# LanceZPF/loongx

Hardware: AMD Instinct MI355X
Metric: edited images/s @512x512, 28-step Flux denoise (higher is better)
Workload: dtype bf16

## Files before the change

loongx_amd/csrc/gemm4.h:

```cpp
#pragma once
#include "gemm_common.h"

namespace {

constexpr int G4_STAGE = 256 * BK * 2 + BN * BK * 2;
constexpr int G4_LDS = 2 * G4_STAGE;
constexpr int G4_PLD = 132;
static_assert(G4_LDS <= 160 * 1024 && 4 * 2 * 16 * G4_PLD * 4 <= G4_LDS, "LDS budget / epilogue patches");

#ifdef LX_G4_PROBE
__device__ unsigned long long lx_g4_probe_buf[8192 * 8];
#define G4_STAMP(k) if (threadIdx.x == 0 && blockIdx.x < 8192) { asm volatile("s_waitcnt lgkmcnt(0)" ::: "memory"); lx_g4_probe_buf[blockIdx.x * 8 + (k)] = __builtin_amdgcn_s_memtime(); }
#else
#define G4_STAMP(k)
#endif


template <bool SPLIT, bool F16 = false, int NP = 2>
__global__ __launch_bounds__(G4_THREADS) void lx_gemm4_kernel(const GemmArgs args, const int sk_full, const int sk_parts, float* __restrict__ sk_slots,
                                                              int* __restrict__ sk_flags, int* __restrict__ sk_err) {
#if defined(__HIP_DEVICE_COMPILE__)
  __shared__ __attribute__((aligned(1024))) char smem[G4_LDS];
  constexpr int BM = 256, A_BYTES = BM * BK * 2;
  const int pid = blockIdx.x;
  G4_STAMP(0)
  const int total = args.tile_start[MAX_SUB];
  int lid, part = 0;
  if (pid < sk_full) {
    const int q = sk_full >> 3, r = sk_full & 7;
    const int xcd = pid & 7, inx = pid >> 3;
    lid = (xcd < r ? xcd * (q + 1) : r * (q + 1) + (xcd - r) * q) + inx;
  } else {
    const int r = pid - sk_full;
    lid = sk_full + r / NP;
    part = r % NP;
  }
  (void)total;
  const bool split_tile = pid >= sk_full && sk_parts >= 2;
  const int g = tile_group(args, lid);
  lx_gemm_desc P = args.p[g];
  int tm, tn;
  tile_coords<BM>(P, lid - args.tile_start[g], tm, tn);
  const int tid = threadIdx.x, lane = tid & 63;
  const int wave = __builtin_amdgcn_readfirstlane(tid >> 6);
  const int wm = wave >> 1, wn = wave & 1, l15 = lane & 15, lq = lane >> 4;
  int m0 = tm * BM, n0 = tn * BN;
  int M = P.M, N = P.N;
  const int K = P.K;
  const bool w_tiled = (P.epilogue & LX_W_TILED) != 0;
  const int nk1 = K / BK;
  const int nkt = SPLIT ? nk1 * max(P.k_segs, 1) : nk1;
  const int kt_begin = !split_tile ? 0 : NP == 2 ? (part ? nkt >> 1 : 0) : (part * nkt) / NP;
  const int kt_end = !split_tile ? nkt : NP == 2 ? (part ? nkt : nkt >> 1) : ((part + 1) * nkt) / NP;

  uint32_t aoff[8], woff[8];
  {
    const int rsub = lane >> 3, pslot = lane & 7;
#pragma unroll
    for (int j = 0; j < 8; ++j) {
      const int row = (j * 4 + wave) * 8 + rsub;
      const int lslot = pslot ^ ((row >> 1) & 7);
      aoff[j] = (uint32_t)((min(m0 + row, M - 1) - m0) * P.lda + lslot * 8) * 2u;
      woff[j] = w_tiled ? (uint32_t)((j * 4 + wave) * 512 + lane * 8) * 2u : (uint32_t)((min(n0 + row, N - 1) - n0) * P.ldw + lslot * 8) * 2u;
    }
  }
  const __bf16* a_org = (const __bf16*)P.A + (size_t)m0 * P.lda;
  const int kw_tiles = SPLIT && P.k_segs == 3 ? 2 * nk1 : nk1;
  const __bf16* w_org = w_tiled ? (const __bf16*)P.W + ((size_t)tn * kw_tiles) * (BN * BK) : (const __bf16*)P.W + (size_t)n0 * P.ldw;
  const lx_rsrc_t rs_a = lx_make_rsrc(a_org), rs_w = lx_make_rsrc(w_org);
  const int w_kstride_b = (w_tiled ? BN * BK : BK) * 2;
  const int a_lo_b = SPLIT ? P.a_lo_off * 2 : 0;
  auto a_soff = [&](int t) -> int {
    if constexpr (!SPLIT) return t * (BK * 2);
    else {
      const int seg = t >= 2 * nk1 ? 2 : (t >= nk1 ? 1 : 0);
      return (t - seg * nk1) * (BK * 2) + (seg == 1 ? a_lo_b : 0);
    }
  };
  auto w_soff = [&](int t) -> int {
    if constexpr (!SPLIT) return t * w_kstride_b;
    else {
      const int seg = t >= 2 * nk1 ? 2 : (t >= nk1 ? 1 : 0);
      return (t - seg * nk1 + (seg == 2 ? nk1 : 0)) * w_kstride_b;
    }
  };
  auto piece = [&](int p_, int a_so, int w_so, int stage) {
    if (p_ < 8) lx_buf_to_lds(rs_a, (lptr_t)(smem + stage * G4_STAGE + (p_ * 4 + wave) * 1024), aoff[p_], a_so);
    else lx_buf_to_lds(rs_w, (lptr_t)(smem + stage * G4_STAGE + A_BYTES + ((p_ - 8) * 4 + wave) * 1024), woff[p_ - 8], w_so);
  };
  int a_ad[2], w_ad[2];
  {
    const int ar = wm * 128 + l15, wr = wn * 128 + l15;
#pragma unroll
    for (int ks = 0; ks < 2; ++ks) {
      a_ad[ks] = ar * 128 + (((ks * 4 + lq) ^ ((ar >> 1) & 7)) * 16);
      w_ad[ks] = A_BYTES + wr * 128 + (((ks * 4 + lq) ^ ((wr >> 1) & 7)) * 16);
    }
  }
  f32x4 acc[8][8];
#pragma unroll
  for (int i = 0; i < 8; ++i)
#pragma unroll
    for (int j = 0; j < 8; ++j) acc[i][j] = f32x4{0.f, 0.f, 0.f, 0.f};
  bf16x8 af[2][8], wf[2][8];
  auto rd = [&](int stage, int ks, int idx) {
    const char* base = smem + stage * G4_STAGE;
    if (idx < 8) wf[ks][idx] = *(const bf16x8*)(base + w_ad[ks] + idx * 2048);
    else af[ks][idx - 8] = *(const bf16x8*)(base + a_ad[ks] + (idx - 8) * 2048);
  };
  auto mm = [&](int ks, int n_) {
    const int j = n_ >> 3, i = n_ & 7;
    if constexpr (F16) asm volatile("v_mfma_f32_16x16x32_f16 %0, %1, %2, %0" : "+a"(acc[i][j]) : "v"(wf[ks][j]), "v"(af[ks][i]));
    else asm volatile("v_mfma_f32_16x16x32_bf16 %0, %1, %2, %0" : "+a"(acc[i][j]) : "v"(wf[ks][j]), "v"(af[ks][i]));
  };
#define G4_SB() __builtin_amdgcn_sched_barrier(0)
  const bool has_lora = P.lora_t != nullptr && kt_begin == 0;
  u32x2 lu[8], lt[8][4];
  if (has_lora) {
    const int R = P.lora_r, nsplit = P.lora_nsplit;
    const int toff = R * min(n0 / max(P.lora_mod_cols, 1), P.lora_toff_max);
    const int rk = min(2 * lq, R - 2);
#pragma unroll
    for (int j = 0; j < 8; ++j) lu[j] = *(const u32x2*)(P.lora_up + (size_t)min(n0 + wn * 128 + j * 16 + l15, N - 1) * R + rk);
#pragma unroll
    for (int i = 0; i < 8; ++i) {
      const float* tp = P.lora_t + (size_t)min(m0 + wm * 128 + i * 16 + l15, M - 1) * P.lora_ldt + toff + rk;
#pragma unroll
      for (int q = 0; q < 4; ++q) lt[i][q] = *(const u32x2*)(tp + (size_t)min(q, nsplit - 1) * P.lora_split_stride);
    }
  }
  {
    const int t1 = min(kt_begin + 1, kt_end - 1);
    const int a0 = a_soff(kt_begin), w0 = w_soff(kt_begin), a1 = a_soff(t1), w1 = w_soff(t1);
#pragma unroll
    for (int p_ = 0; p_ < 16; ++p_) piece(p_, a0, w0, 0);
#pragma unroll
    for (int p_ = 0; p_ < 16; ++p_) piece(p_, a1, w1, 1);
  }
  asm volatile("s_waitcnt vmcnt(16)" ::: "memory");
  __builtin_amdgcn_s_barrier();
  G4_SB();
  G4_STAMP(1)
#pragma unroll
  for (int x = 0; x < 16; ++x) rd(0, 0, x);
  if (has_lora) {
    const int R = P.lora_r, nsplit = P.lora_nsplit;
    const bool live = 2 * lq < R;
    auto frag_u = [&](u32x2 v) {
      const float a = live ? __uint_as_float(v[0]) : 0.f, b = live ? __uint_as_float(v[1]) : 0.f;
      const uint16_t ah = f32_to_bf16(a), bh = f32_to_bf16(b);
      const uint16_t al = f32_to_bf16(a - bf16_to_f32(ah)), bl = f32_to_bf16(b - bf16_to_f32(bh));
      const u32x4 w = {(uint32_t)ah * 0x10001u, (uint32_t)al * 0x10001u, (uint32_t)bh * 0x10001u, (uint32_t)bl * 0x10001u};
      return __builtin_bit_cast(bf16x8, w);
    };
    auto frag_t = [&](float a, float b) {
      a = live ? a : 0.f; b = live ? b : 0.f;
      const uint16_t ah = f32_to_bf16(a), bh = f32_to_bf16(b);
      const uint32_t pa = (uint32_t)ah | ((uint32_t)f32_to_bf16(a - bf16_to_f32(ah)) << 16);
      const uint32_t pb = (uint32_t)bh | ((uint32_t)f32_to_bf16(b - bf16_to_f32(bh)) << 16);
      const u32x4 w = {pa, pa, pb, pb};
      return __builtin_bit_cast(bf16x8, w);
    };
    bf16x8 uf[8], tf[8];
#pragma unroll
    for (int j = 0; j < 8; ++j) uf[j] = frag_u(lu[j]);
#pragma unroll
    for (int i = 0; i < 8; ++i) {
      float a = __uint_as_float(lt[i][0][0]), b = __uint_as_float(lt[i][0][1]);
#pragma unroll
      for (int q = 1; q < 4; ++q)
        if (q < nsplit) { a += __uint_as_float(lt[i][q][0]); b += __uint_as_float(lt[i][q][1]); }
      tf[i] = frag_t(a, b);
    }
#pragma unroll
    for (int j = 0; j < 8; ++j)
#pragma unroll
      for (int i = 0; i < 8; ++i) acc[i][j] = __builtin_amdgcn_mfma_f32_16x16x32_bf16(uf[j], tf[i], acc[i][j], 0, 0, 0);
    asm volatile("s_nop 15\n s_nop 7" ::: "memory");
  }
  asm volatile("s_waitcnt lgkmcnt(0)" ::: "memory");
  G4_STAMP(2)
  int c = 0;
  for (int kt = kt_begin; kt < kt_end; ++kt) {
    const int n = c ^ 1;
    const int kt2 = min(kt + 2, kt_end - 1);
    const int a_so2 = a_soff(kt2), w_so2 = w_soff(kt2);
#pragma unroll
    for (int m = 0; m < 64; ++m) {
      if (m == 16) {
        G4_SB();
        asm volatile("s_waitcnt lgkmcnt(0)" ::: "memory");
        __builtin_amdgcn_s_barrier();
        G4_SB();
      }
      mm(0, m); G4_SB();
      if (m < 16) { rd(c, 1, m); G4_SB(); }
      if (m >= 16 && (m - 16) % 6 == 0) { piece((m - 16) / 6, a_so2, w_so2, c); G4_SB(); }
    }
#pragma unroll
    for (int m = 0; m < 64; ++m) {
      if (m == 43) {
        G4_SB();
        asm volatile("s_waitcnt vmcnt(16)" ::: "memory");
        __builtin_amdgcn_s_barrier();
        G4_SB();
      }
      mm(1, m); G4_SB();
      if (m < 40 && m % 5 == 0) { piece(8 + m / 5, a_so2, w_so2, c); G4_SB(); }
      if (m >= 43 && m < 59) { rd(n, 0, m - 43); G4_SB(); }
    }
    asm volatile("s_waitcnt lgkmcnt(0)" ::: "memory");
    c = n;
  }
#undef G4_SB
  G4_STAMP(3)
  asm volatile("s_nop 15\n s_nop 7\n s_waitcnt vmcnt(0)" ::: "memory");
  __syncthreads();
  G4_STAMP(4)

  const float* partner = nullptr;
  const float* partner2 = nullptr;
  float* my_slot = nullptr;
  if (split_tile) {
    my_slot = sk_slots + (size_t)(pid - sk_full) * SK_SLOT_FLOATS;
    if constexpr (NP == 2) {
      partner = sk_slots + (size_t)((pid - sk_full) ^ 1) * SK_SLOT_FLOATS;
    } else {
      const int gb = (pid - sk_full) - part;
      partner = sk_slots + (size_t)(gb + (part + 1) % NP) * SK_SLOT_FLOATS;
      partner2 = sk_slots + (size_t)(gb + (part + 2) % NP) * SK_SLOT_FLOATS;
    }
  }
  auto pld4 = [&](size_t off_floats, const float* from) {
    const u32x4 v = __builtin_amdgcn_raw_buffer_load_b128(lx_make_rsrc(from), (int)(off_floats * 4), 0, PAIR_AUX_SC1);
    return f32x4{__uint_as_float(v[0]), __uint_as_float(v[1]), __uint_as_float(v[2]), __uint_as_float(v[3])};
  };
  const int lm0 = wm * 128, ln0 = wn * 128;
  auto exchange = [&]() {
    asm volatile("s_waitcnt vmcnt(0)" ::: "memory");
    __syncthreads();
    __builtin_amdgcn_fence(__ATOMIC_RELEASE, "workgroup");
    if (tid == 0) {
      const int me = pid - sk_full, other = NP == 2 ? (me ^ 1) : (me - part + (part + 1) % NP), other2 = me - part + (part + 2) % NP;
      bool ok = __hip_atomic_load(sk_err, __ATOMIC_RELAXED, __HIP_MEMORY_SCOPE_AGENT) == 0;
      if (ok) {
        if (!(sk_parts == 3 && part == 1))
          __hip_atomic_store(sk_flags + me, NP - 1, __ATOMIC_RELAXED, __HIP_MEMORY_SCOPE_AGENT);
        int spins = 0;
        while (__hip_atomic_load(sk_flags + other, __ATOMIC_RELAXED, __HIP_MEMORY_SCOPE_AGENT) == 0) {
          __builtin_amdgcn_s_sleep(1);
          if (++spins > (1 << 20)) { ok = false; break; }
        }
        if constexpr (NP == 3) {
          while (ok && __hip_atomic_load(sk_flags + other2, __ATOMIC_RELAXED, __HIP_MEMORY_SCOPE_AGENT) == 0) {
            __builtin_amdgcn_s_sleep(1);
            if (++spins > (1 << 20)) { ok = false; break; }
          }
        }
        if (ok) {
          if constexpr (NP == 2) __hip_atomic_store(sk_flags + other, 0, __ATOMIC_RELAXED, __HIP_MEMORY_SCOPE_AGENT);
          else {
            __hip_atomic_fetch_add(sk_flags + other, -1, __ATOMIC_RELAXED, __HIP_MEMORY_SCOPE_AGENT);
            __hip_atomic_fetch_add(sk_flags + other2, -1, __ATOMIC_RELAXED, __HIP_MEMORY_SCOPE_AGENT);
          }
        } else __hip_atomic_store(sk_err, 1, __ATOMIC_RELAXED, __HIP_MEMORY_SCOPE_AGENT);
      }
    }
    __syncthreads();
    G4_STAMP(6)
    __builtin_amdgcn_fence(__ATOMIC_ACQUIRE, "workgroup");
  };

  const int epi = P.epilogue & 0xff;
  const bool do_gelu = (P.epilogue & LX_EPI_GELU) != 0;
  const int mw0 = m0 + wm * 128, nw0 = n0 + wn * 128;
  float* patch = (float*)smem + wave * (2 * 16 * G4_PLD);
  const bool bf16_out = epi == LX_EPI_STORE_BF16;
  const int c8 = (lane & 15) * 8, c4 = (lane & 31) * 4;
  const int ncol = nw0 + (bf16_out ? c8 : c4);
  const bool col_ok = ncol < N;
  f32x4 bias0 = {0.f, 0.f, 0.f, 0.f}, bias1 = {0.f, 0.f, 0.f, 0.f};
  if (P.bias && col_ok) {
    bias0 = *(const f32x4*)(P.bias + ncol);
    if (bf16_out) bias1 = *(const f32x4*)(P.bias + ncol + 4);
  }
  asm volatile("s_waitcnt vmcnt(0)" : "+v"(bias0), "+v"(bias1)::"memory");
  const bool gelu0 = do_gelu && ncol >= P.gelu_col_start;
  const int m_base = args.m_base[g];
  static_assert(!(F16 && SPLIT), "fp16 operands exclude the split-bf16 mode");
  float f16_mx = 0.f;
  const bool qkv_tile = (P.epilogue & LX_EPI_QKV) != 0 && n0 < 3 * P.qkv_d;
  const int qkind = qkv_tile ? n0 / P.qkv_d : -1;
  f32x4 nw0v = {1.f, 1.f, 1.f, 1.f}, nw1v = {1.f, 1.f, 1.f, 1.f};
  if (qkv_tile && qkind != 1) {
    const float* nwp = (qkind == 2 ? P.qkv_norm_q : P.qkv_norm_k) + c8;
    nw0v = *(const f32x4*)nwp; nw1v = *(const f32x4*)(nwp + 4);
    asm volatile("s_waitcnt vmcnt(0)" : "+v"(nw0v), "+v"(nw1v)::"memory");
  }
  auto put = [&](auto ic_) {
    constexpr int i = decltype(ic_)::value;
    float* pt = patch + (i & 1) * (16 * G4_PLD);
    asm volatile("" : "+a"(acc[i][0]), "+a"(acc[i][1]), "+a"(acc[i][2]), "+a"(acc[i][3]), "+a"(acc[i][4]), "+a"(acc[i][5]), "+a"(acc[i][6]), "+a"(acc[i][7]));
#pragma unroll
    for (int j = 0; j < 8; ++j) *(f32x4*)(pt + l15 * G4_PLD + j * 16 + 4 * lq) = acc[i][j];
  };
  auto park = [&](auto ic_, auto nx_) {
    constexpr int i = decltype(ic_)::value, nx = decltype(nx_)::value;
    const float* pt = patch + (i & 1) * (16 * G4_PLD);
    __builtin_amdgcn_wave_barrier();
    if constexpr (nx >= 0) { if (mw0 + nx * 16 < M) put(std::integral_constant<int, nx>{}); }
    __builtin_amdgcn_sched_barrier(0);
    if (mw0 + i * 16 >= M) return;
    const lx_rsrc_t rs_slot = lx_make_rsrc(my_slot);
#pragma unroll
    for (int t = 0; t < 8; ++t) {
      const int row = t * 2 + (lane >> 5);
      const f32x4 v = *(const f32x4*)(pt + row * G4_PLD + c4);
      __builtin_amdgcn_raw_buffer_store_b128(u32x4{__float_as_uint(v[0]), __float_as_uint(v[1]), __float_as_uint(v[2]), __float_as_uint(v[3])}, rs_slot,
                                             (int)(((size_t)(wm * 128 + i * 16 + row) * 256 + wn * 128 + c4) * 4), 0, PAIR_AUX_SC1);
    }
  };
  auto block = [&](auto ic_, auto nx_) {
    constexpr int i = decltype(ic_)::value, nx = decltype(nx_)::value;
    const int mb = mw0 + i * 16;
    if (mb >= M) return;
    const float* pt = patch + (i & 1) * (16 * G4_PLD);
    f32x4 res[8], gat[8];
    if (epi == LX_EPI_RESID_F32 && !qkv_tile) {
      const int rpb = P.rows_per_batch;
#pragma unroll
      for (int t = 0; t < 8; ++t) {
        const int m = mb + t * 2 + (lane >> 5);
        if (m < M && col_ok) {
          res[t] = *(const f32x4*)((const float*)P.C + (size_t)m * P.ldc + ncol);
          if (P.gate) gat[t] = *(const f32x4*)(P.gate + (size_t)((m_base + m) / rpb) * P.gate_ld + ncol);
        }
      }
    }
    __builtin_amdgcn_wave_barrier();
    if constexpr (nx >= 0) { if (mw0 + nx * 16 < M) put(std::integral_constant<int, nx>{}); }
    __builtin_amdgcn_sched_barrier(0);
    if (partner) {
      f32x4 pa[4][2], pb[4][2];
#pragma unroll
      for (int t = 0; t < 4; ++t) {
        const size_t po = (size_t)(lm0 + i * 16 + t * 4 + (lane >> 4)) * 256 + ln0 + c8;
        pa[t][0] = pld4(po, partner); pa[t][1] = pld4(po + 4, partner);
        if constexpr (NP == 3) { pb[t][0] = pld4(po, partner2); pb[t][1] = pld4(po + 4, partner2); }
      }
      float* pw = patch + (i & 1) * (16 * G4_PLD);
#pragma unroll
      for (int t = 0; t < 4; ++t) {
        float* q_ = pw + (t * 4 + (lane >> 4)) * G4_PLD + c8;
        f32x4 v0 = *(const f32x4*)q_, v1 = *(const f32x4*)(q_ + 4);
#pragma unroll
        for (int c_ = 0; c_ < 4; ++c_) { v0[c_] += pa[t][0][c_]; v1[c_] += pa[t][1][c_]; }
        if constexpr (NP == 3) {
#pragma unroll
          for (int c_ = 0; c_ < 4; ++c_) { v0[c_] += pb[t][0][c_]; v1[c_] += pb[t][1][c_]; }
        }
        *(f32x4*)q_ = v0; *(f32x4*)(q_ + 4) = v1;
      }
      __builtin_amdgcn_wave_barrier();
    }
    if (qkv_tile) {
      const int D = P.qkv_d, L = P.rows_per_batch, H = D >> 7;
      const int gm = m_base + mb, b = gm / L, p0 = gm - b * L;
      const int h = (nw0 - qkind * D) >> 7;
      if (qkind == 1) {
        const int gk = lane & 1;
        float e[4][8];
#pragma unroll
        for (int t = 0; t < 4; ++t)
#pragma unroll
          for (int k = 0; k < 8; ++k) {
            const int rk = qkv_vt_interleave(gk * 8 + k), dk = t * 32 + (lane >> 1);
            e[t][k] = pt[rk * G4_PLD + dk];
          }
#pragma unroll
        for (int t = 0; t < 4; ++t) {
          const int d = t * 32 + (lane >> 1);
          const float bd = P.bias ? P.bias[nw0 + d] : 0.f;
          u32x4 o = {pack_bf16x2(e[t][0] + bd, e[t][1] + bd), pack_bf16x2(e[t][2] + bd, e[t][3] + bd), pack_bf16x2(e[t][4] + bd, e[t][5] + bd),
                     pack_bf16x2(e[t][6] + bd, e[t][7] + bd)};
          *(u32x4*)((uint16_t*)P.qkv_vt + ((size_t)(b * H + h) * 128 + d) * P.qkv_vt_ld + P.qkv_vt_pos0 + p0 + gk * 8) = o;
        }
      } else {
        uint16_t* const out = (qkind == 0 && P.qkv_k) ? (uint16_t*)P.qkv_k : (uint16_t*)P.C;
        const int out_ld = (qkind == 0 && P.qkv_k) ? P.qkv_k_ld : P.ldc;
        f32x4 cs[4][2], pv[4][2];
#pragma unroll
        for (int t = 0; t < 4; ++t) {
          const float* rp = P.qkv_rope + (size_t)(p0 + t * 4 + (lane >> 4)) * 128 + c8;
          cs[t][0] = *(const f32x4*)rp; cs[t][1] = *(const f32x4*)(rp + 4);
        }
#pragma unroll
        for (int t = 0; t < 4; ++t) {
          const int row = t * 4 + (lane >> 4);
          pv[t][0] = *(const f32x4*)(pt + row * G4_PLD + c8); pv[t][1] = *(const f32x4*)(pt + row * G4_PLD + c8 + 4);
        }
        float yy[4][8];
#pragma unroll
        for (int t = 0; t < 4; ++t) {
          f32x4 v0 = pv[t][0], v1 = pv[t][1];
          float ss = 0.f;
#pragma unroll
          for (int c_ = 0; c_ < 4; ++c_) { v0[c_] += bias0[c_]; v1[c_] += bias1[c_]; ss = __builtin_fmaf(v0[c_], v0[c_], ss); ss = __builtin_fmaf(v1[c_], v1[c_], ss); }
#ifdef LX_G4_ROW16_SHFL
          ss += __shfl_xor(ss, 1, 64); ss += __shfl_xor(ss, 2, 64); ss += __shfl_xor(ss, 4, 64); ss += __shfl_xor(ss, 8, 64);
#else
          ss = row16_sum(ss);
#endif
          const float r = rsqrtf(ss * (1.0f / 128.0f) + 1e-6f);
          float x[8];
          float (&y)[8] = yy[t];
#pragma unroll
          for (int c_ = 0; c_ < 4; ++c_) { x[c_] = v0[c_] * r * nw0v[c_]; x[4 + c_] = v1[c_] * r * nw1v[c_]; }
#pragma unroll
          for (int q = 0; q < 4; ++q) {
            const float co = q < 2 ? cs[t][0][2 * q] : cs[t][1][2 * q - 4], si = q < 2 ? cs[t][0][2 * q + 1] : cs[t][1][2 * q - 3];
            y[2 * q] = x[2 * q] * co - x[2 * q + 1] * si;
            y[2 * q + 1] = x[2 * q + 1] * co + x[2 * q] * si;
          }
        }
#pragma unroll
        for (int t = 0; t < 4; ++t) {
          const int m = mb + t * 4 + (lane >> 4);
          const float (&y)[8] = yy[t];
          u32x4 o = {pack_bf16x2(y[0], y[1]), pack_bf16x2(y[2], y[3]), pack_bf16x2(y[4], y[5]), pack_bf16x2(y[6], y[7])};
          if (m < M) *(u32x4*)(out + (size_t)m * out_ld + ncol) = o;
        }
      }
      return;
    }
    if (bf16_out) {
      f32x4 pv[4][2];
#pragma unroll
      for (int t = 0; t < 4; ++t) {
        const int row = t * 4 + (lane >> 4);
        pv[t][0] = *(const f32x4*)(pt + row * G4_PLD + c8); pv[t][1] = *(const f32x4*)(pt + row * G4_PLD + c8 + 4);
      }
#pragma unroll
      for (int t = 0; t < 4; ++t) {
        const int row = t * 4 + (lane >> 4), m = mb + row;
        f32x4 v0 = pv[t][0], v1 = pv[t][1];
        if (m < M && col_ok) {
#pragma unroll
          for (int c_ = 0; c_ < 4; ++c_) { v0[c_] += bias0[c_]; v1[c_] += bias1[c_]; }
          if (gelu0) { v0 = gelu_tanh4(v0); v1 = gelu_tanh4(v1); }
          u32x4 o = {pack_op16x2<F16>(v0[0], v0[1], f16_mx), pack_op16x2<F16>(v0[2], v0[3], f16_mx), pack_op16x2<F16>(v1[0], v1[1], f16_mx),
                     pack_op16x2<F16>(v1[2], v1[3], f16_mx)};
          *(u32x4*)((uint16_t*)P.C + (size_t)m * P.ldc + ncol) = o;
          if constexpr (SPLIT) {
            if (P.epilogue & LX_EPI_SPLIT_BF16) {
              float r[8];
#pragma unroll
              for (int c_ = 0; c_ < 4; ++c_) {
                r[c_] = v0[c_] - bf16_to_f32(f32_to_bf16(v0[c_]));
                r[4 + c_] = v1[c_] - bf16_to_f32(f32_to_bf16(v1[c_]));
              }
              u32x4 ol = {pack_bf16x2(r[0], r[1]), pack_bf16x2(r[2], r[3]), pack_bf16x2(r[4], r[5]), pack_bf16x2(r[6], r[7])};
              *(u32x4*)((uint16_t*)P.C + (size_t)m * P.ldc + ncol + P.c_lo_off) = ol;
            }
          }
        }
      }
    } else {
      f32x4 pv[8];
#pragma unroll
      for (int t = 0; t < 8; ++t) pv[t] = *(const f32x4*)(pt + (t * 2 + (lane >> 5)) * G4_PLD + c4);
      if (epi == LX_EPI_RESID_F32) {
        asm volatile("s_waitcnt vmcnt(0)" ::: "memory");
#pragma unroll
        for (int t = 0; t < 8; ++t) asm volatile("" : "+v"(res[t]), "+v"(gat[t]));
      }
#pragma unroll
      for (int t = 0; t < 8; ++t) {
        const int row = t * 2 + (lane >> 5), m = mb + row;
        f32x4 v = pv[t];
        if (m < M && col_ok) {
#pragma unroll
          for (int c_ = 0; c_ < 4; ++c_) v[c_] += bias0[c_];
          if (gelu0) v = gelu_tanh4(v);
          if (epi == LX_EPI_RESID_F32) {
            f32x4 o = res[t];
            if (P.gate) {
#pragma unroll
              for (int c_ = 0; c_ < 4; ++c_) o[c_] = __builtin_fmaf(gat[t][c_], v[c_], o[c_]);
            } else {
#pragma unroll
              for (int c_ = 0; c_ < 4; ++c_) o[c_] += v[c_];
            }
            v = o;
          }
          *(f32x4*)((float*)P.C + (size_t)m * P.ldc + ncol) = v;
        }
      }
    }
  };
#define G4_B(I, NX) block(std::integral_constant<int, I>{}, std::integral_constant<int, NX>{})
#define G4_K(I, NX) park(std::integral_constant<int, I>{}, std::integral_constant<int, NX>{})
  if (!split_tile) {
    if (mw0 < M) put(std::integral_constant<int, 0>{});
    G4_B(0, 1); G4_B(1, 2); G4_B(2, 3); G4_B(3, 4); G4_B(4, 5); G4_B(5, 6); G4_B(6, 7); G4_B(7, -1);
  } else if constexpr (NP == 2) {
    if (part == 0) {
      if (mw0 + 64 < M) put(std::integral_constant<int, 4>{});
      G4_K(4, 5); G4_K(5, 6); G4_K(6, 7); G4_K(7, 0);
      exchange();
      G4_B(0, 1); G4_B(1, 2); G4_B(2, 3); G4_B(3, -1);
    } else {
      if (mw0 < M) put(std::integral_constant<int, 0>{});
      G4_K(0, 1); G4_K(1, 2); G4_K(2, 3); G4_K(3, 4);
      exchange();
      G4_B(4, 5); G4_B(5, 6); G4_B(6, 7); G4_B(7, -1);
    }
  } else {
    if (part == 0) {
      if (mw0 + 48 < M) put(std::integral_constant<int, 3>{});
      G4_K(3, 4); G4_K(4, 5); G4_K(5, 6); G4_K(6, 7); G4_K(7, 0);
      exchange();
      G4_B(0, 1); G4_B(1, 2); G4_B(2, -1);
    } else if (part == 1) {
      if (mw0 < M) put(std::integral_constant<int, 0>{});
      G4_K(0, 1); G4_K(1, 2); G4_K(2, 7); G4_K(7, 6); G4_K(6, 3);
      exchange();
      G4_B(3, 4); G4_B(4, 5); G4_B(5, -1);
    } else {
      if (mw0 < M) put(std::integral_constant<int, 0>{});
      G4_K(0, 1); G4_K(1, 2); G4_K(2, 3); G4_K(3, 4); G4_K(4, 5); G4_K(5, 6);
      exchange();
      G4_B(6, 7); G4_B(7, -1);
    }
  }
#undef G4_B
#undef G4_K
  if constexpr (F16) { if (bf16_out && !qkv_tile) report_f16_overflow(f16_mx, P.f16_ovf); }
  asm volatile("s_waitcnt vmcnt(0)" ::: "memory");
  G4_STAMP(5)
#endif
}


}
```

Before: 1.066.

## Prefetch epilogue operands before main loop and preload first block's residual/rope

Moves the bias, qk-norm weight, V-transpose bias and per-batch gate loads ahead of the K loop so their latency hides behind the MFMA work. It also issues the first epilogue block's residual or rope loads before the post-loop barrier. Per-row gate loads are replaced with at most two hoisted gate vectors plus a fallback for tiles spanning more batches. This costs extra live VGPRs across the main loop, which could raise register pressure or spill.

Result: no change. 1.071 (median of 6 runs) (+0.5%).

```diff
diff --git a/loongx_amd/csrc/gemm4.h b/loongx_amd/csrc/gemm4.h
--- a/loongx_amd/csrc/gemm4.h
+++ b/loongx_amd/csrc/gemm4.h
@@ -127,6 +127,43 @@
       const float* tp = P.lora_t + (size_t)min(m0 + wm * 128 + i * 16 + l15, M - 1) * P.lora_ldt + toff + rk;
 #pragma unroll
       for (int q = 0; q < 4; ++q) lt[i][q] = *(const u32x2*)(tp + (size_t)min(q, nsplit - 1) * P.lora_split_stride);
+    }
+  }
+  const int epi = P.epilogue & 0xff;
+  const int mw0 = m0 + wm * 128, nw0 = n0 + wn * 128;
+  const bool bf16_out = epi == LX_EPI_STORE_BF16;
+  const int c8 = (lane & 15) * 8, c4 = (lane & 31) * 4;
+  const int ncol = nw0 + (bf16_out ? c8 : c4);
+  const bool col_ok = ncol < N;
+  const int m_base = args.m_base[g];
+  const bool qkv_tile = (P.epilogue & LX_EPI_QKV) != 0 && n0 < 3 * P.qkv_d;
+  const int qkind = qkv_tile ? n0 / P.qkv_d : -1;
+  f32x4 bias0 = {0.f, 0.f, 0.f, 0.f}, bias1 = {0.f, 0.f, 0.f, 0.f};
+  if (P.bias && col_ok) {
+    bias0 = *(const f32x4*)(P.bias + ncol);
+    if (bf16_out) bias1 = *(const f32x4*)(P.bias + ncol + 4);
+  }
+  f32x4 nw0v = {1.f, 1.f, 1.f, 1.f}, nw1v = {1.f, 1.f, 1.f, 1.f};
+  if (qkv_tile && qkind != 1) {
+    const float* nwp = (qkind == 2 ? P.qkv_norm_q : P.qkv_norm_k) + c8;
+    nw0v = *(const f32x4*)nwp; nw1v = *(const f32x4*)(nwp + 4);
+  }
+  f32x4 vtb = {0.f, 0.f, 0.f, 0.f};
+  if (qkv_tile && qkind == 1 && P.bias) {
+#pragma unroll
+    for (int t = 0; t < 4; ++t) vtb[t] = P.bias[nw0 + t * 32 + (lane >> 1)];
+  }
+  f32x4 gate0 = {0.f, 0.f, 0.f, 0.f}, gate1 = {0.f, 0.f, 0.f, 0.f};
+  int gate_edge = 0, gate_edge2 = 0;
+  bool gate_far = false;
+  if (epi == LX_EPI_RESID_F32 && !qkv_tile && P.gate && mw0 < M) {
+    const int rpb = P.rows_per_batch, b0 = (m_base + mw0) / rpb, mlast = min(mw0 + 127, M - 1);
+    gate_edge = mw0 + min(rpb - (m_base + mw0 - b0 * rpb), 256);
+    gate_edge2 = gate_edge + min(rpb, 256);
+    gate_far = mlast >= gate_edge2;
+    if (col_ok) {
+      gate0 = *(const f32x4*)(P.gate + (size_t)b0 * P.gate_ld + ncol);
+      if (mlast >= gate_edge) gate1 = *(const f32x4*)(P.gate + (size_t)(b0 + 1) * P.gate_ld + ncol);
     }
   }
   {
@@ -214,8 +251,26 @@
   }
 #undef G4_SB
   G4_STAMP(3)
-  asm volatile("s_nop 15\n s_nop 7\n s_waitcnt vmcnt(0)" ::: "memory");
-  __syncthreads();
+  asm volatile("s_waitcnt vmcnt(0)" : "+v"(bias0), "+v"(bias1), "+v"(nw0v), "+v"(nw1v), "+v"(vtb), "+v"(gate0), "+v"(gate1)::"memory");
+  const int blk_first = !split_tile ? 0 : NP == 2 ? part * 4 : part * 3;
+  const int mb_first = mw0 + blk_first * 16;
+  f32x4 pre[8];
+  if (mb_first < M) {
+    if (epi == LX_EPI_RESID_F32 && !qkv_tile) {
+#pragma unroll
+      for (int t = 0; t < 8; ++t) pre[t] = *(const f32x4*)((const float*)P.C + (size_t)min(mb_first + t * 2 + (lane >> 5), M - 1) * P.ldc + (col_ok ? ncol : n0));
+    } else if (qkv_tile && qkind != 1) {
+      const int gm = m_base + mb_first, p0 = gm - (gm / P.rows_per_batch) * P.rows_per_batch;
+#pragma unroll
+      for (int t = 0; t < 4; ++t) {
+        const float* rp = P.qkv_rope + (size_t)(p0 + t * 4 + (lane >> 4)) * 128 + c8;
+        pre[2 * t] = *(const f32x4*)rp; pre[2 * t + 1] = *(const f32x4*)(rp + 4);
+      }
+    }
+  }
+  asm volatile("s_nop 15\n s_nop 7" ::: "memory");
+  __builtin_amdgcn_s_barrier();
+  asm volatile("" ::: "memory");
   G4_STAMP(4)
 
   const float* partner = nullptr;
@@ -271,32 +326,11 @@
     __builtin_amdgcn_fence(__ATOMIC_ACQUIRE, "workgroup");
   };
 
-  const int epi = P.epilogue & 0xff;
   const bool do_gelu = (P.epilogue & LX_EPI_GELU) != 0;
-  const int mw0 = m0 + wm * 128, nw0 = n0 + wn * 128;
   float* patch = (float*)smem + wave * (2 * 16 * G4_PLD);
-  const bool bf16_out = epi == LX_EPI_STORE_BF16;
-  const int c8 = (lane & 15) * 8, c4 = (lane & 31) * 4;
-  const int ncol = nw0 + (bf16_out ? c8 : c4);
-  const bool col_ok = ncol < N;
-  f32x4 bias0 = {0.f, 0.f, 0.f, 0.f}, bias1 = {0.f, 0.f, 0.f, 0.f};
-  if (P.bias && col_ok) {
-    bias0 = *(const f32x4*)(P.bias + ncol);
-    if (bf16_out) bias1 = *(const f32x4*)(P.bias + ncol + 4);
-  }
-  asm volatile("s_waitcnt vmcnt(0)" : "+v"(bias0), "+v"(bias1)::"memory");
   const bool gelu0 = do_gelu && ncol >= P.gelu_col_start;
-  const int m_base = args.m_base[g];
   static_assert(!(F16 && SPLIT), "fp16 operands exclude the split-bf16 mode");
   float f16_mx = 0.f;
-  const bool qkv_tile = (P.epilogue & LX_EPI_QKV) != 0 && n0 < 3 * P.qkv_d;
-  const int qkind = qkv_tile ? n0 / P.qkv_d : -1;
-  f32x4 nw0v = {1.f, 1.f, 1.f, 1.f}, nw1v = {1.f, 1.f, 1.f, 1.f};
-  if (qkv_tile && qkind != 1) {
-    const float* nwp = (qkind == 2 ? P.qkv_norm_q : P.qkv_norm_k) + c8;
-    nw0v = *(const f32x4*)nwp; nw1v = *(const f32x4*)(nwp + 4);
-    asm volatile("s_waitcnt vmcnt(0)" : "+v"(nw0v), "+v"(nw1v)::"memory");
-  }
   auto put = [&](auto ic_) {
     constexpr int i = decltype(ic_)::value;
     float* pt = patch + (i & 1) * (16 * G4_PLD);
@@ -320,20 +354,20 @@
                                              (int)(((size_t)(wm * 128 + i * 16 + row) * 256 + wn * 128 + c4) * 4), 0, PAIR_AUX_SC1);
     }
   };
-  auto block = [&](auto ic_, auto nx_) {
+  auto block = [&](auto ic_, auto nx_, auto first_) {
     constexpr int i = decltype(ic_)::value, nx = decltype(nx_)::value;
+    constexpr bool first = decltype(first_)::value;
     const int mb = mw0 + i * 16;
     if (mb >= M) return;
     const float* pt = patch + (i & 1) * (16 * G4_PLD);
-    f32x4 res[8], gat[8];
+    f32x4 res[8];
     if (epi == LX_EPI_RESID_F32 && !qkv_tile) {
-      const int rpb = P.rows_per_batch;
 #pragma unroll
       for (int t = 0; t < 8; ++t) {
         const int m = mb + t * 2 + (lane >> 5);
         if (m < M && col_ok) {
-          res[t] = *(const f32x4*)((const float*)P.C + (size_t)m * P.ldc + ncol);
-          if (P.gate) gat[t] = *(const f32x4*)(P.gate + (size_t)((m_base + m) / rpb) * P.gate_ld + ncol);
+          if constexpr (first) res[t] = pre[t];
+          else res[t] = *(const f32x4*)((const float*)P.C + (size_t)m * P.ldc + ncol);
         }
       }
     }
@@ -380,7 +414,7 @@
 #pragma unroll
         for (int t = 0; t < 4; ++t) {
           const int d = t * 32 + (lane >> 1);
-          const float bd = P.bias ? P.bias[nw0 + d] : 0.f;
+          const float bd = vtb[t];
           u32x4 o = {pack_bf16x2(e[t][0] + bd, e[t][1] + bd), pack_bf16x2(e[t][2] + bd, e[t][3] + bd), pack_bf16x2(e[t][4] + bd, e[t][5] + bd),
                      pack_bf16x2(e[t][6] + bd, e[t][7] + bd)};
           *(u32x4*)((uint16_t*)P.qkv_vt + ((size_t)(b * H + h) * 128 + d) * P.qkv_vt_ld + P.qkv_vt_pos0 + p0 + gk * 8) = o;
@@ -391,8 +425,11 @@
         f32x4 cs[4][2], pv[4][2];
 #pragma unroll
         for (int t = 0; t < 4; ++t) {
-          const float* rp = P.qkv_rope + (size_t)(p0 + t * 4 + (lane >> 4)) * 128 + c8;
-          cs[t][0] = *(const f32x4*)rp; cs[t][1] = *(const f32x4*)(rp + 4);
+          if constexpr (first) { cs[t][0] = pre[2 * t]; cs[t][1] = pre[2 * t + 1]; }
+          else {
+            const float* rp = P.qkv_rope + (size_t)(p0 + t * 4 + (lane >> 4)) * 128 + c8;
+            cs[t][0] = *(const f32x4*)rp; cs[t][1] = *(const f32x4*)(rp + 4);
+          }
         }
 #pragma unroll
         for (int t = 0; t < 4; ++t) {
@@ -472,7 +509,7 @@
       if (epi == LX_EPI_RESID_F32) {
         asm volatile("s_waitcnt vmcnt(0)" ::: "memory");
 #pragma unroll
-        for (int t = 0; t < 8; ++t) asm volatile("" : "+v"(res[t]), "+v"(gat[t]));
+        for (int t = 0; t < 8; ++t) asm volatile("" : "+v"(res[t]));
       }
 #pragma unroll
       for (int t = 0; t < 8; ++t) {
@@ -485,8 +522,10 @@
           if (epi == LX_EPI_RESID_F32) {
             f32x4 o = res[t];
             if (P.gate) {
-#pragma unroll
-              for (int c_ = 0; c_ < 4; ++c_) o[c_] = __builtin_fmaf(gat[t][c_], v[c_], o[c_]);
+              f32x4 gt = m < gate_edge ? gate0 : gate1;
+              if (gate_far && m >= gate_edge2) gt = *(const f32x4*)(P.gate + (size_t)((m_base + m) / P.rows_per_batch) * P.gate_ld + ncol);
+#pragma unroll
+              for (int c_ = 0; c_ < 4; ++c_) o[c_] = __builtin_fmaf(gt[c_], v[c_], o[c_]);
             } else {
 #pragma unroll
               for (int c_ = 0; c_ < 4; ++c_) o[c_] += v[c_];
@@ -498,42 +537,44 @@
       }
     }
   };
-#define G4_B(I, NX) block(std::integral_constant<int, I>{}, std::integral_constant<int, NX>{})
+#define G4_B(I, NX) block(std::integral_constant<int, I>{}, std::integral_constant<int, NX>{}, std::false_type{})
+#define G4_F(I, NX) block(std::integral_constant<int, I>{}, std::integral_constant<int, NX>{}, std::true_type{})
 #define G4_K(I, NX) park(std::integral_constant<int, I>{}, std::integral_constant<int, NX>{})
   if (!split_tile) {
     if (mw0 < M) put(std::integral_constant<int, 0>{});
-    G4_B(0, 1); G4_B(1, 2); G4_B(2, 3); G4_B(3, 4); G4_B(4, 5); G4_B(5, 6); G4_B(6, 7); G4_B(7, -1);
+    G4_F(0, 1); G4_B(1, 2); G4_B(2, 3); G4_B(3, 4); G4_B(4, 5); G4_B(5, 6); G4_B(6, 7); G4_B(7, -1);
   } else if constexpr (NP == 2) {
     if (part == 0) {
       if (mw0 + 64 < M) put(std::integral_constant<int, 4>{});
       G4_K(4, 5); G4_K(5, 6); G4_K(6, 7); G4_K(7, 0);
       exchange();
-      G4_B(0, 1); G4_B(1, 2); G4_B(2, 3); G4_B(3, -1);
+      G4_F(0, 1); G4_B(1, 2); G4_B(2, 3); G4_B(3, -1);
     } else {
       if (mw0 < M) put(std::integral_constant<int, 0>{});
       G4_K(0, 1); G4_K(1, 2); G4_K(2, 3); G4_K(3, 4);
       exchange();
-      G4_B(4, 5); G4_B(5, 6); G4_B(6, 7); G4_B(7, -1);
+      G4_F(4, 5); G4_B(5, 6); G4_B(6, 7); G4_B(7, -1);
     }
   } else {
     if (part == 0) {
       if (mw0 + 48 < M) put(std::integral_constant<int, 3>{});
       G4_K(3, 4); G4_K(4, 5); G4_K(5, 6); G4_K(6, 7); G4_K(7, 0);
       exchange();
-      G4_B(0, 1); G4_B(1, 2); G4_B(2, -1);
+      G4_F(0, 1); G4_B(1, 2); G4_B(2, -1);
     } else if (part == 1) {
       if (mw0 < M) put(std::integral_constant<int, 0>{});
       G4_K(0, 1); G4_K(1, 2); G4_K(2, 7); G4_K(7, 6); G4_K(6, 3);
       exchange();
-      G4_B(3, 4); G4_B(4, 5); G4_B(5, -1);
+      G4_F(3, 4); G4_B(4, 5); G4_B(5, -1);
     } else {
       if (mw0 < M) put(std::integral_constant<int, 0>{});
       G4_K(0, 1); G4_K(1, 2); G4_K(2, 3); G4_K(3, 4); G4_K(4, 5); G4_K(5, 6);
       exchange();
-      G4_B(6, 7); G4_B(7, -1);
+      G4_F(6, 7); G4_B(7, -1);
     }
   }
 #undef G4_B
+#undef G4_F
 #undef G4_K
   if constexpr (F16) { if (bf16_out && !qkv_tile) report_f16_overflow(f16_mx, P.f16_ovf); }
   asm volatile("s_waitcnt vmcnt(0)" ::: "memory");
```
